# cmower/optas

Measured on AMD Instinct MI355X. Metric: MPC solves/sec (KUKA 7-DoF, T=50), higher is better.
Workload: dtype f64; 1 GPU; figure_eight_plan T=50 KUKA LWR end_effector_ball (BASELINE configs[1]) x 262144 perturbed instances per GPU (qc0 + U(-0.1,0.1)^7, seed=qc), solved to reduced-gradient tol 1e-08, max_iter 300; batch_per_gpu=262144, global_batch=262144, T=50, parallelism=dp1 (instances sharded, one RCCL broadcast of constants), rccl_world=1, hessian=hybrid, streams_per_gpu=2

## Files before the change

### optas_amd/csrc/oh_api.hip

```cpp
#include <dlfcn.h>
#include <hip/hip_runtime.h>
#include <rccl/rccl.h>

#include <chrono>
#include <cmath>
#include <cstdio>
#include <cstdlib>
#include <cstring>
#include <array>
#include <map>
#include <mutex>
#include <string>
#include <thread>
#include <utility>
#include <vector>

#include "oh_kernels.h"
#include "oh_jit.h"
#include "oh_rnea.h"

static thread_local std::string g_err;

static int fail(int code, const std::string& msg) {
  g_err = msg;
  return code;
}

#define HIPCHK(expr)                                                                                   \
  do {                                                                                                 \
    hipError_t _e = (expr);                                                                            \
    if (_e != hipSuccess) {                                                                            \
      return fail(OH_ERR_HIP, std::string(#expr) + ": " + hipGetErrorString(_e));                     \
    }                                                                                                  \
  } while (0)

#define OH_PINNED_STAGE_BYTES (256 * 1024)

struct Sched {
  int compaction = 1;
  int compact_carry = 1;
  int tail_vel_threshold = 1 << 30;
  int lg_split = 1;
  int tail_vel = 1;
  int compact_sort = 1;
  double compact_frac = 0.97;
  double compact_frac_restart = 0.9;
  int tail_threshold = 16384;
  int sparse_check_below = 2048;
  int fuse_couple = 1;
  int free_pcr_max = 1536;
  int specialize = OH_SPECIALIZE_AUTO;
  int tq_check = 4;
  std::array<double, 4> inv_saved{1.0, 16384.0, 1.0, -2.0};
};

struct oh_handle;
struct LastSolve {
  struct Part { const oh_handle* q; int n; };
  int B = 0;
  std::vector<Part> parts;
  bool pipe_cache = false;
};

// ... 57 lines not shown
  int cap_B = 0;
  FigBuffers D{};
  FigParams P{};
  void* pool = nullptr;
  size_t pool_bytes = 0;
  LastSolve last;
  void* stage = nullptr;
  size_t stage_bytes = 0;
  bool profiling = false;
  std::vector<hipEvent_t> prof_events;
  double timing[8] = {0, 0, 0, 0, 0, 0, 0, 0};
  double timing_couple = 0;
  double rejects = 0;
  double tail_iters = 0;
  int* h_flag = nullptr;
  std::vector<oh_handle*> peers;
  double* d_pipe_mult = nullptr;
  size_t pipe_mult_cap = 0;
  bool is_peer = false;
  Sched sch;
  int specialize_min_B = 4096;
  const FigSpec* spec = nullptr;
  bool spec_failed = false;
  bool spec_cache_checked = false;
  const FkSpec* fk_spec = nullptr;
  bool fk_spec_failed = false;
  int specialize_min_units = 1 << 16;
  double spec_seconds = 0.0;
  std::vector<int> prof_tags;
  std::map<std::string, double> opt;
  std::vector<int> t_op, t_a, t_b, t_rows;
  std::vector<double> t_c;
  oh_tape_desc t_desc{};
};

extern "C" void oh_destroy(oh_handle* h);
extern "C" int oh_specialize(oh_handle* h);
static bool spec_applies(const oh_handle* h);
static bool spec_tail_vel_applies(const oh_handle* h);
static int specialize_fk(oh_handle* h);
extern "C" const char* oh_last_error(void) { return g_err.c_str(); }
extern "C" const char* oh_version(void) { return "optas_hip 0.2 (gfx950)"; }
extern "C" int oh_abi_version(void) { return OH_ABI_VERSION; }

struct OptDoc { const char* name; double dflt; };
static constexpr OptDoc OPT_TABLE[] = {
// ... 17 lines not shown
  static_assert(ROW >= 0, "optv: the option is not in OPT_TABLE");
  return ROW;
}
static double opt_value(const oh_handle* h, const OptDoc& d) {
  const auto it = h->opt.find(d.name);
  return it == h->opt.end() ? d.dflt : it->second;
}
#define optv(h, name) opt_value(h, OPT_TABLE[known_opt<opt_row(name)>()])
static double batch_invariant(const oh_handle* h) {
  const auto it = h->opt.find("batch_invariant");
  return it == h->opt.end() ? 0.0 : it->second;
}
struct FieldOpt {
  const char* name;
  int Sched::*i;
  double Sched::*d = nullptr;
  bool flag = false;
  double get(const Sched& s) const { return d ? s.*d : s.*i; }
  void set(Sched& s, const double v) const { if (d) s.*d = v; else s.*i = flag ? v != 0.0 : (int)v; }
};
static const FieldOpt FIELD_OPTS[] = {
    {"tail_threshold", &Sched::tail_threshold}, {"free_pcr_max", &Sched::free_pcr_max}, {"compaction", &Sched::compaction, nullptr, true},
    {"compact_frac", nullptr, &Sched::compact_frac}, {"compact_sort", &Sched::compact_sort}, {"compact_carry", &Sched::compact_carry},
    {"tail_vel", &Sched::tail_vel}, {"lg_split", &Sched::lg_split}, {"tail_vel_threshold", &Sched::tail_vel_threshold},
    {"fuse_couple", &Sched::fuse_couple, nullptr, true}, {"sparse_check_below", &Sched::sparse_check_below}, {"specialize", &Sched::specialize},
    {"tq_check", &Sched::tq_check},
};
static const FieldOpt* field_opt(const std::string& name) {
  for (const FieldOpt& f : FIELD_OPTS)
    if (name == f.name) return &f;
  return nullptr;
}
static int tape_configure(oh_handle* h);
static int set_option_impl(oh_handle* h, const std::string& name, double v) {
  Sched& sc = h->sch;
  if (name == "compact_frac") sc.compact_frac = sc.compact_frac_restart = v;
  else if (name == "specialize") sc.specialize = v == 0.0 ? OH_SPECIALIZE_NEVER : (v == 1.0 ? OH_SPECIALIZE_ALWAYS : OH_SPECIALIZE_AUTO);
  else if (name == "tq_check") sc.tq_check = v >= 1.0 ? (int)v : 1;
  else if (name == "batch_invariant") {
    const bool was = batch_invariant(h) != 0.0;
    h->opt[name] = v;
    if (v != 0.0 && !was) {
      sc.inv_saved = {sc.compaction ? 1.0 : 0.0, (double)sc.tail_threshold, (double)sc.tail_vel, h->opt.count("free_persist") ? h->opt["free_persist"] : -2.0};
      sc.compaction = false; sc.tail_threshold = 0; sc.tail_vel = 0; h->opt["free_persist"] = 0;
    } else if (v == 0.0 && was) {
      sc.compaction = sc.inv_saved[0] != 0.0; sc.tail_threshold = (int)sc.inv_saved[1]; sc.tail_vel = (int)sc.inv_saved[2];
// ... 909 lines not shown
  if (c.n_chain < 1 || c.n_chain > OH_MAX_CHAIN || c.ndof < c.n_chain || c.ndof > OH_MAX_CHAIN)
    return fail(OH_ERR_INVALID, "oh_set_constants: bad n_chain/ndof");
  for (int k = 0; k < c.n_chain; ++k) {
    if (c.jtype[k] != 0 && c.jtype[k] != 1) return fail(OH_ERR_INVALID, "oh_set_constants: joint type not supported");
    if (c.qidx[k] < 0 || c.qidx[k] >= c.ndof) return fail(OH_ERR_INVALID, "oh_set_constants: qidx out of range");
  }
  if (c.ndof != h->desc.ndof) return fail(OH_ERR_INVALID, "oh_set_constants: chain.ndof != desc.ndof");
  return OH_OK;
}

static void drop_peers(oh_handle* h) {
  h->last = LastSolve{};
  if (h->is_peer) return;
  for (oh_handle* p : h->peers) oh_destroy(p);
  h->peers.clear();
}

static void adopt_chain(oh_handle* h, const oh_chain& c) {
  drop_peers(h);
  h->chain_host = c;
  h->have_chain = true;
  h->spec = nullptr;
  h->spec_failed = false;
  h->spec_cache_checked = false;
  h->fk_spec = nullptr;
  h->fk_spec_failed = false;
}

extern "C" int oh_set_constants(oh_handle* h, const oh_chain* chain) {
  if (!h || !chain) return fail(OH_ERR_INVALID, "oh_set_constants: null argument");
  int rc = validate_chain(h, *chain);
  if (rc) return rc;
  HIPCHK(hipMemcpy(h->d_chain, chain, sizeof(oh_chain), hipMemcpyHostToDevice));
  adopt_chain(h, *chain);
  return OH_OK;
}

extern "C" int oh_set_constants_device(oh_handle* h, const void* d_chain, size_t nbytes) {
  if (!h || !d_chain) return fail(OH_ERR_INVALID, "oh_set_constants_device: null argument");
  if (nbytes != sizeof(oh_chain)) return fail(OH_ERR_INVALID, "oh_set_constants_device: nbytes != sizeof(oh_chain)");
  oh_chain tmp;
  HIPCHK(hipMemcpy(&tmp, d_chain, sizeof(oh_chain), hipMemcpyDeviceToHost));
  int rc = validate_chain(h, tmp);
  if (rc) return rc;
  HIPCHK(hipMemcpy(h->d_chain, d_chain, sizeof(oh_chain), hipMemcpyDeviceToDevice));
  adopt_chain(h, tmp);
// ... 535 lines not shown
  const bool tail_vel = r.guarded && (GP.vel || GP.limits) && GP.n_links == 0 && h->sch.tail_vel;
  const bool tail_ok = (h->desc.T - P.t0 <= 64) && h->sch.tail_threshold > 0 && (!r.guarded || tail_vel) && !r.lead;
  const int tail_threshold = tail_vel ? h->sch.tail_vel_threshold : h->sch.tail_threshold;
  if (tail_ok && r.B <= tail_threshold) {
    if (!launch_tail(h, r, tail_vel, 0)) return fail(OH_ERR_INVALID, "oh_solve_device: no persistent kernel for this handle (ndof / rows)");
    return OH_OK;
  }
  const bool lg_split = r.guarded && h->sch.lg_split && GP.n_links == 0, lg_spec = lg_split && h->spec && spec_tail_vel_applies(h);
  const bool couple_vel = !P.zc && r.guarded && GP.vel, couple = !P.zc && !couple_vel;
  const bool carry = h->sch.compaction && h->sch.compact_carry && (size_t)h->desc.T * ((N - 3) * (N - 2) / 2) >= 22 && !r.guarded && !r.lead;
  const double inv_frac = optv(h, "invariant_compact_frac");
  const bool inv_move = r.invariant && !r.lead && inv_frac > 0.0, restart = h->sch.compaction && !r.lead, restart_moves = r.guarded && optv(h, "compact_move_all") != 0.0;
  int nrun = -1, carry_pending = 0;
  for (int it = 0; it < r.hard_cap; ++it) {
    if (nrun >= 0)
      if (const int rc = mark(h, r, 0, 3)) return rc;
    const int slot = it & 1;
    if (lg_split) {
      if (!(lg_spec && oh_spec_launch_eval(*h->spec, s, P, D, slot, 1) == hipSuccess)) oh_launch_eval_locked_guarded(s, N, P, D, GP, GB, slot, 1);
      oh_launch_eval_locked_guarded(s, N, P, D, GP, GB, slot, 2);
    } else if (r.guarded) oh_launch_eval_locked_guarded(s, N, P, D, GP, GB, slot, 0);
    else if (r.lead) oh_launch_eval_lead(s, N, P, D, slot);
    else if (carry_pending > 0) {
      launch_eval(h, r, slot, 1);
      if (const int rc = mark(h, r, 4)) return rc;
      finalize(h, r, 1);
      oh_launch_scan_running(s, D, h->sch.compact_sort);
      oh_launch_carry(s, N, P, D, 0, 0, slot);
      oh_launch_carry(s, N, P, D, 1, carry_pending, slot);
      std::swap(D.q[slot], D.q_spare[0]);
      std::swap(D.q[1 - slot], D.q_spare[1]);
      if (P.hessian != OH_HESSIAN_GAUSS_NEWTON || P.zc) std::swap(D.Gfull[1 - slot], D.G_spare);
      D.B = carry_pending;
      carry_pending = 0;
      ++r.compactions;
      if (const int rc = mark(h, r, 0)) return rc;
      launch_eval(h, r, slot, 2);
    } else launch_eval(h, r, slot, 0);
    if (const int rc = mark(h, r, 1)) return rc;
    if (couple_vel) oh_launch_couple_vel(s, N, P, D, GP, GB, slot);
    else if (couple) oh_launch_couple(s, N, P, D, slot);
    const bool check = check_after(h, r, it, tail_ok);
    if (const int rc = mark(h, r, 3)) return rc;
    if (r.guarded) oh_launch_step_locked_guarded(s, N, P, D, GP, GB, slot);
    else oh_launch_step(s, N, P, D, slot);
    if (const int rc = mark(h, r, 2)) return rc;
    ++r.launched;
    if (const int rc = look(h, check, &nrun)) return rc;
    if (nrun == 0) break;
    if (tail_ok && nrun > 0 && nrun <= tail_threshold) {
      if (const int rc = compact_batch(h, r, nrun, (it + 1) & 1, false)) return rc;
// ... 876 lines not shown
```

### optas_amd/csrc/oh_figure8_kernels.h

```cpp
#pragma once
#include "oh_figure8_units.h"

template <int N>
__device__ void retract_block(const FigParams& P, const FigBuffers& D, const int slot) {
  eval_unit<N, false, false, EVAL_RETRACT_ONLY>(P, D, slot, blockIdx.x * blockDim.x + threadIdx.x, blockIdx.y + P.t0);
}
template <int N>
__device__ void finalize_block(const FigParams& P, const FigBuffers& D, const int only_done, double* __restrict__ f, double* __restrict__ kkt, int* __restrict__ iters,
                               int* __restrict__ status) {
  finalize_unit<N>(P, D, only_done, nullptr, f, kkt, iters, status, blockIdx.x * blockDim.x + threadIdx.x, blockIdx.y);
}
template <int N, bool ZC = false>
__device__ void evalb_block(const FigParams& P, const FigBuffers& D, const int slot) {
  if constexpr (ZC) {
    if (blockIdx.x == 0 && threadIdx.x == 0) *D.n_running = 0;
    const int Tn = P.T - P.t0;
    const int w = blockIdx.x;
    const int chunk = w / (8 * Tn), r = w - chunk * 8 * Tn;
    eval_unit<N, false, false, EVAL_ONLY, true>(P, D, slot, (chunk * 8 + (r & 7)) * blockDim.x + threadIdx.x, (r >> 3) + P.t0);
  } else {
    eval_unit<N, false, false, EVAL_ONLY, false>(P, D, slot, blockIdx.x * blockDim.x + threadIdx.x, blockIdx.y + P.t0);
  }
}

OH_DEV double bcast(const double v, const int lane) {
  int lo = __double2loint(v), hi = __double2hiint(v);
  lo = __builtin_amdgcn_readlane(lo, lane);
  hi = __builtin_amdgcn_readlane(hi, lane);
// ... 523 lines not shown
```

### optas_amd/csrc/oh_figure8_units.h

```cpp
#pragma once
#include "oh_figure8.h"

#define IDX(t, K, k) (((size_t)(t) * (K) + (k)) * Bp + b)
#define KNOT(arr, t, K) rowbuf((arr) + (size_t)(t) * (K) * (size_t)Bp)
#define RB(k) ((unsigned)(k) * rowB)



template <int N>
OH_DEV void setup_unit(const FigParams& P, const FigBuffers& D, const double* __restrict__ x0, const double* __restrict__ pin, const int b, const int tt) {
  const int Bp = D.Bp;
  if (b >= D.B) {
    if (b < Bp && tt == 0) D.status[b] = OH_STATUS_CONVERGED;
    return;
  }
  const oh_chain* ch = D.chain;
  double qc[N];
#pragma unroll
  for (int j = 0; j < N; ++j) qc[j] = pin[(size_t)b * P.np + j];
#pragma unroll
  for (int j = 0; j < N; ++j) {
    const double v = (tt < P.t0) ? qc[j] : x0[(size_t)b * P.nx + (size_t)tt * N + j];
    D.q[0][IDX(tt, N, j)] = v;
    D.q[1][IDX(tt, N, j)] = (tt < P.t0) ? qc[j] : 0.0;
  }
  if (ch->has_lead) D.lead[(size_t)tt * Bp + b] = pin[(size_t)b * P.np + N + 1 + tt];
  if (tt != 0) return;
  double R[9], p[3], z[N][3], pj[N][3];
// ... 34 lines not shown
  D.feas[b] = 0.0;
}

#ifndef OH_CHAIN
#define OH_CHAIN(D) ((D).chain)
#endif
#ifndef OH_RETRACT_PREFETCH
#define OH_RETRACT_PREFETCH 0
#endif
#ifndef OH_EVALB_PREFETCH_G
#define OH_EVALB_PREFETCH_G 1
#endif
#ifndef OH_ZC_EARLY
#define OH_ZC_EARLY 1
#endif
template <int N>
OH_DEV void load_householder(const double* __restrict__ Vs, const int Bp, const int b, const int t, double (&V)[3][N]) {
#pragma unroll
  for (int m = 0; m < 3; ++m)
#pragma unroll
    for (int k = 0; k < N; ++k) V[m][k] = (k < m) ? 0.0 : Vs[IDX(t, HV_ROWS(N), HV_OFF(N, m) + k - m)];
}

template <int N, bool GUARD = false, bool LEAD = false, int MODE = EVAL_FUSED, bool ZC = false, bool SPH = true>
OH_DEV void eval_unit(const FigParams& P, const FigBuffers& D, const int slot, const int b, const int t, const GuardParams* GPp = nullptr,
                      const GuardBuffers* GBp = nullptr) {
  static_assert(!ZC || (MODE == EVAL_ONLY && !GUARD && !LEAD), "the folded coupling belongs to the plain batched evaluation");
  constexpr int NZ = N - 3;
  constexpr int NP = NZ * (NZ + 1) / 2;
  const int Bp = D.Bp;
  if (b >= D.B) return;
  const int cur = 1 - slot;
  const int status_b = D.status[b], skip_b = D.skip[b], first_b = D.first[b];
  const bool asis = (MODE == EVAL_RETRACT_ONLY && !GUARD) ? D.polish[b] == 2 : false;
  const double stat_b = D.stat[b], pred_b = D.pred[b];
  constexpr bool EARLY = MODE == EVAL_ONLY || OH_RETRACT_PREFETCH;
  double Rc[9], pc[3];
  if constexpr (EARLY) {
#pragma unroll
    for (int i = 0; i < 3; ++i) pc[i] = D.ref[(size_t)i * Bp + b];
#pragma unroll
    for (int i = 0; i < 9; ++i) Rc[i] = D.ref[(size_t)(3 + i) * Bp + b];
  }
  double q[N], e_tgt[3] = {0.0, 0.0, 0.0};
  double sm_zc = 0.0;
  double zs[NZ], Vc[3][N], mdlc[3 + 3 * NZ];
  double Gpre[N];
  constexpr bool PRE_G = OH_EVALB_PREFETCH_G && MODE == EVAL_ONLY && !GUARD;
  if constexpr (MODE == EVAL_ONLY) {
#pragma unroll
    for (int j = 0; j < N; ++j) q[j] = D.q[slot][IDX(t, N, j)];
    if constexpr (PRE_G) {
      if (P.hessian != OH_HESSIAN_GAUSS_NEWTON) {
#pragma unroll
        for (int k = 0; k < N; ++k) Gpre[k] = D.Gfull[cur][IDX(t, N, k)];
      }
    }
  } else if constexpr (OH_RETRACT_PREFETCH) {
#pragma unroll
    for (int a = 0; a < NZ; ++a) zs[a] = D.zstep[IDX(t, NZ, a)];
    load_householder<N>(D.Z[cur], Bp, b, t, Vc);
#pragma unroll
    for (int j = 0; j < N; ++j) q[j] = D.q[cur][IDX(t, N, j)];
#pragma unroll
    for (int i = 0; i < 3 + 3 * NZ; ++i) mdlc[i] = D.mdl[cur][IDX(t, MDL_ROWS(N), i)];
  }
  double cpl_zc[N];
  if constexpr (ZC && OH_ZC_EARLY) {
    const double* __restrict__ qs = D.q[slot];
    const bool lastk = (t == P.T - 1);
    double qm[N], qp[N];
#pragma unroll
    for (int k = 0; k < N; ++k) {
      qm[k] = qs[IDX(t - 1, N, k)];
      qp[k] = lastk ? 0.0 : qs[IDX(t + 1, N, k)];
    }
    oh_fence(q[N - 1]);
    oh_fence(Rc[8]);
    oh_fence(qp[N - 1]);
    const double kap2 = 2.0 * P.kappa;
#pragma unroll
    for (int k = 0; k < N; ++k) {
      const double dm = q[k] - qm[k];
      sm_zc += dm * dm;
      double c = kap2 * dm;
      if (!lastk) c -= kap2 * (qp[k] - q[k]);
      cpl_zc[k] = c;
    }
  } else if constexpr (EARLY) {
    oh_fence(q[N - 1]);
    oh_fence(Rc[8]);
  }
  if (status_b >= 0 || skip_b) return;
  const bool first = first_b != 0;
  if constexpr (MODE != EVAL_ONLY) {
    if (first) {
#pragma unroll
      for (int j = 0; j < N; ++j) q[j] = D.q[slot][IDX(t, N, j)];
    } else {
      if constexpr (!OH_RETRACT_PREFETCH) {
#pragma unroll
        for (int a = 0; a < NZ; ++a) zs[a] = D.zstep[IDX(t, NZ, a)];
        load_householder<N>(D.Z[cur], Bp, b, t, Vc);
#pragma unroll
        for (int j = 0; j < N; ++j) q[j] = D.q[cur][IDX(t, N, j)];
#pragma unroll
        for (int i = 0; i < 3 + 3 * NZ; ++i) mdlc[i] = D.mdl[cur][IDX(t, MDL_ROWS(N), i)];
      }
      double Zc[N][NZ];
      z_from_householder<N>(Vc, Zc);
#pragma unroll
      for (int j = 0; j < N; ++j) {
        double v = q[j];
#pragma unroll
        for (int a = 0; a < NZ; ++a) v += Zc[j][a] * zs[a];
        q[j] = asis ? q[j] : v;
      }
#pragma unroll
      for (int m = 0; m < 3; ++m) {
        double v = mdlc[m];
#pragma unroll
        for (int a = 0; a < NZ; ++a) v += mdlc[3 + m * NZ + a] * zs[a];
        e_tgt[m] = v;
      }
    }
  }
  if constexpr (!EARLY) {
#pragma unroll
    for (int i = 0; i < 3; ++i) pc[i] = D.ref[(size_t)i * Bp + b];
#pragma unroll
    for (int i = 0; i < 9; ++i) Rc[i] = D.ref[(size_t)(3 + i) * Bp + b];
  }
  double Gprev[N];
  const bool fresh = first_b == 1;
  bool exact = (P.hessian == OH_HESSIAN_EXACT) || (P.hessian == OH_HESSIAN_HYBRID && !fresh && stat_b <= P.hyb_switch);
  if constexpr (GUARD) {
    if (SPH && GPp->n_links > 0) exact = false;
  }
  const bool have_G = exact && !fresh;
#pragma unroll
  for (int k = 0; k < N; ++k) Gprev[k] = 0.0;

  double phi, cv, g[N], Dr[NP], Z[N][NZ];
  struct Hooks {
    double* __restrict__ qo;
    double* __restrict__ go;
    double* __restrict__ vo;
    const double* __restrict__ Gc;
    int Bp, b, t;
    OH_DEV void q_final(const double (&qv)[N]) const {
      if constexpr (!GUARD && MODE != EVAL_ONLY) {
#pragma unroll
        for (int j = 0; j < N; ++j) qo[IDX(t, N, j)] = qv[j];
      }
    }
    OH_DEV void g_final(const double (&gv)[N]) const {
      if constexpr (ZC && OH_ZC_EARLY) {
#pragma unroll
        for (int k = 0; k < N; ++k) Go[IDX(t, N, k)] = gv[k] + cpl[k];
      } else if constexpr (ZC) {
        double sm = 0.0;
#pragma unroll
        for (int k = 0; k < N; ++k) {
          const double q0 = qr[k];
          const double dm = q0 - qs[IDX(t - 1, N, k)];
          sm += dm * dm;
          double Gk = gv[k] + kap2 * dm;
          if (!last) Gk -= kap2 * (qs[IDX(t + 1, N, k)] - q0);
          Go[IDX(t, N, k)] = Gk;
        }
        *smo = sm;
      } else if constexpr (!GUARD) {
#pragma unroll
        for (int k = 0; k < N; ++k) go[IDX(t, N, k)] = gv[k];
      }
    }
    OH_DEV void v_final(const double (&Vv)[3][N]) const {
#pragma unroll
      for (int m = 0; m < 3; ++m)
#pragma unroll
        for (int k = m; k < N; ++k) vo[IDX(t, HV_ROWS(N), HV_OFF(N, m) + k - m)] = Vv[m][k];
    }
    const double* Gp;
    OH_DEV void load_G(const double (&)[N], double (&G)[N]) const {
#pragma unroll
      for (int k = 0; k < N; ++k) G[k] = PRE_G ? Gp[k] : Gc[IDX(t, N, k)];
    }
    const double* __restrict__ qs;
    const double* qr;
    double* __restrict__ Go;
    double* smo;
    double kap2;
    bool last;
    const double* cpl;
  };
  const Hooks hooks{D.q[slot], D.g[slot], D.Z[slot], D.Gfull[cur], Bp, b, t, Gpre, D.q[slot], q, D.Gfull[slot], &sm_zc, 2.0 * P.kappa, t == P.T - 1, cpl_zc};
  double e_new[3], JZ_new[3][NZ];
  const double tol_r = (first_b == 2 || asis) ? 1e300 : retract_tol(P, !first, pred_b, stat_b);
  if constexpr (LEAD)
    eval_knot<N, true, Hooks, MODE>(OH_CHAIN(D), P, t, q, pc, Rc, exact, have_G, Gprev, phi, cv, g, Dr, Z, !first, e_tgt, tol_r, e_new, JZ_new,
                                    D.lead[(size_t)t * Bp + b], hooks);
  else eval_knot<N, false, Hooks, MODE>(OH_CHAIN(D), P, t, q, pc, Rc, exact, have_G, Gprev, phi, cv, g, Dr, Z, !first, e_tgt, tol_r, e_new, JZ_new, 0.0, hooks);
  if constexpr (MODE == EVAL_RETRACT_ONLY) return;
#pragma unroll
  for (int m = 0; m < 3; ++m) {
    D.mdl[slot][IDX(t, MDL_ROWS(N), m)] = e_new[m];
#pragma unroll
    for (int a = 0; a < NZ; ++a) D.mdl[slot][IDX(t, MDL_ROWS(N), 3 + m * NZ + a)] = JZ_new[m][a];
  }
  if constexpr (GUARD) {
    const GuardParams& GP = *GPp;
    const GuardBuffers& GB = *GBp;
    const bool upd = GB.outer[b] != 0;
    const double rho_old = GB.rho[b];
    const double rho = upd ? GB.rho_next[b] : rho_old;
    const double irho = 1.0 / rho, i2rho = 1.0 / (2.0 * rho);
    double psi = 0.0, meas = 0.0, dd[N];
    const int nl = GP.limits ? 2 * N : 0;
#pragma unroll
// ... 866 lines not shown
```

### optas_amd/csrc/oh_jit.h

```cpp
#pragma once
#include <string>
#include <vector>

#include "oh_kernels.h"

struct FigSpec {
  hipModule_t mod = nullptr;
  hipFunction_t retract = nullptr, evalb = nullptr, evalb_zc = nullptr, tail = nullptr, tail_vel = nullptr, finalize = nullptr;
  int n = 0;
  bool from_disk = false;
  double seconds = 0.0;
};
std::string oh_jit_figure8_source(const oh_chain& chain, int N);
int oh_jit_compile_cached(const std::string& src, std::vector<char>* code, bool* from_disk, std::string* err, bool ignore_disk = false);
int oh_jit_figure8(const oh_chain& chain, int N, const FigSpec** out, std::string* err);
bool oh_jit_figure8_cached(const oh_chain& chain, int N);
hipError_t oh_spec_launch_eval(const FigSpec& sp, hipStream_t s, const FigParams& P, const FigBuffers& D, int slot, int part);
hipError_t oh_spec_launch_tail(const FigSpec& sp, hipStream_t s, const FigParams& P, const FigBuffers& D, int slot);
hipError_t oh_spec_launch_finalize(const FigSpec& sp, hipStream_t s, FigParams P, FigBuffers D, int only_done, double* f, double* kkt, int* iters, int* status);
hipError_t oh_spec_launch_tail_vel(const FigSpec& sp, hipStream_t s, FigParams P, FigBuffers D, GuardParams GP, GuardBuffers GB, int slot);
bool oh_spec_kernel_info(const FigSpec& sp, const char* name, OhKernelInfo* out);

bool oh_jit_disk_lookup(const std::string& key_text, const char* prefix, std::vector<char>* code);
void oh_jit_disk_store(const std::string& key_text, const char* prefix, const std::vector<char>& code);
void oh_jit_disk_drop(const std::string& key_text, const char* prefix);

struct FkSpec {
  hipModule_t mod = nullptr;
  hipFunction_t soa = nullptr, aos = nullptr;
  int ndof = 0;
  bool from_disk = false;
// ... 7 lines not shown
```

### optas_amd/csrc/oh_jit.hip

```cpp
#include <hip/hip_runtime.h>
#include <hip/hiprtc.h>
#include <sys/stat.h>
#include <unistd.h>

#include <chrono>
#include <cstdio>
#include <cstdlib>
#include <cstring>
#include <map>
#include <mutex>
#include <string>
#include <vector>

#include "oh_jit.h"
#include "oh_fkjac_unit.h"
#include "oh_jit_headers.h"

namespace {
std::mutex g_mutex;
std::map<unsigned long long, FigSpec*> g_specs;
std::map<unsigned long long, FkSpec*> g_fk_specs;

unsigned long long fnv1a(const std::string& s, unsigned long long h = 1469598103934665603ull) {
  for (unsigned char c : s) {
// ... 151 lines not shown
  char name[96];
  snprintf(name, sizeof name, "%s_%016llx.hsaco", prefix, fnv1a("hiprtc " + std::to_string(major) + "." + std::to_string(minor), fnv1a(key_text)));
  remove((dir + "/" + name).c_str());
}

std::string oh_jit_figure8_source(const oh_chain& chain, int N) {
  std::string s;
  s += "// generated by liboptas_hip (oh_jit.hip): figure-eight evaluation kernels for one kinematic chain\n";
  s += "#include \"oh_types.h\"\n";
  s += "static __device__ constexpr oh_chain oh_spec_chain = " + chain_literal(chain) + ";\n";
  s += "#define OH_CHAIN(D) (&oh_spec_chain)\n";
#ifndef OH_JIT_RETRACT_PREFETCH
#define OH_JIT_RETRACT_PREFETCH 1
#endif
  s += "#define OH_RETRACT_PREFETCH " + std::to_string(OH_JIT_RETRACT_PREFETCH) + "\n";
#ifndef OH_JIT_ZC_EARLY
#define OH_JIT_ZC_EARLY 1
#endif
  s += "#define OH_ZC_EARLY " + std::to_string(OH_JIT_ZC_EARLY) + "\n";
  s += "#include \"oh_platform_gfx950.h\"\n";
  s += "#include \"oh_figure8_kernels.h\"\n";
  const std::string n = std::to_string(N);
  s += "extern \"C\" __global__ __launch_bounds__(256, 2) void oh_spec_retract(FigParams P, FigBuffers D, const int slot) { retract_block<" + n + ">(P, D, slot); }\n";
  s += "extern \"C\" __global__ __launch_bounds__(256, 2) void oh_spec_evalb(FigParams P, FigBuffers D, const int slot) { evalb_block<" + n + ">(P, D, slot); }\n";
  s += "extern \"C\" __global__ __launch_bounds__(256, 2) void oh_spec_evalb_zc(FigParams P, FigBuffers D, const int slot) { evalb_block<" + n + ", true>(P, D, slot); }\n";
  s += "extern \"C\" __global__ __launch_bounds__(64) void oh_spec_tail(FigParams P, FigBuffers D, const int slot) { tail_block<" + n + ">(P, D, slot); }\n";
  s += "extern \"C\" __global__ __launch_bounds__(256) void oh_spec_finalize(FigParams P, FigBuffers D, const int only_done, double* f, double* kkt, int* iters, int* status) { finalize_block<" + n +
       ">(P, D, only_done, f, kkt, iters, status); }\n";
  s += "extern \"C\" __global__ __launch_bounds__(64) void oh_spec_tail_vel(FigParams P, FigBuffers D, GuardParams GP, GuardBuffers GB, const int slot) { tail_block<" + n +
       ", true>(P, D, slot, &GP, &GB); }\n";
  return s;
}

int oh_jit_compile_cached(const std::string& src, std::vector<char>* code, bool* from_disk, std::string* err, bool ignore_disk) {
  const std::string name = cache_name(src);
  const std::string dir = cache_dir();
  *from_disk = false;
  if (ignore_disk && !dir.empty()) remove((dir + "/" + name).c_str());
  if (!ignore_disk && !dir.empty() && read_file(dir + "/" + name, code)) {
    *from_disk = true;
    return 0;
  }
  if (compile(src, code, err)) return 1;
  if (!dir.empty()) {
    mkdirs(dir);
    write_file_atomic(dir + "/" + name, *code);
// ... 22 lines not shown
  const auto t0 = std::chrono::steady_clock::now();
  const std::string src = oh_jit_figure8_source(chain, N);
  int dev = 0;
  hipGetDevice(&dev);
  const unsigned long long key = fnv1a(src) ^ (0x9e3779b97f4a7c15ull * (unsigned long long)(dev + 1));
  std::lock_guard<std::mutex> lk(g_mutex);
  auto it = g_specs.find(key);
  if (it != g_specs.end()) {
    *out = it->second;
    return 0;
  }
  std::vector<char> code;
  bool from_disk = false;
  FigSpec* sp = new FigSpec();
  for (int attempt = 0;; ++attempt) {
    if (oh_jit_compile_cached(src, &code, &from_disk, err, attempt > 0)) {
      delete sp;
      return 1;
    }
    const char* what = nullptr;
    if (hipModuleLoadData(&sp->mod, code.data()) != hipSuccess) what = "hipModuleLoadData";
    else if (hipModuleGetFunction(&sp->retract, sp->mod, "oh_spec_retract") != hipSuccess || hipModuleGetFunction(&sp->evalb, sp->mod, "oh_spec_evalb") != hipSuccess ||
             hipModuleGetFunction(&sp->tail, sp->mod, "oh_spec_tail") != hipSuccess || hipModuleGetFunction(&sp->evalb_zc, sp->mod, "oh_spec_evalb_zc") != hipSuccess ||
             hipModuleGetFunction(&sp->tail_vel, sp->mod, "oh_spec_tail_vel") != hipSuccess || hipModuleGetFunction(&sp->finalize, sp->mod, "oh_spec_finalize") != hipSuccess) {
      what = "hipModuleGetFunction";
      hipModuleUnload(sp->mod);
    }
    if (!what) break;
    (void)hipGetLastError();
    if (from_disk && attempt == 0) continue;
    *err = std::string(what) + " failed for the specialised figure-eight kernels";
    delete sp;
    return 1;
  }
  sp->n = N;
  sp->from_disk = from_disk;
  sp->seconds = std::chrono::duration<double>(std::chrono::steady_clock::now() - t0).count();
  g_specs.emplace(key, sp);
  *out = sp;
  return 0;
}

static hipError_t launch3(hipFunction_t f, dim3 g, dim3 b, hipStream_t s, FigParams P, FigBuffers D, int slot) {
  void* args[] = {&P, &D, &slot};
  return hipModuleLaunchKernel(f, g.x, g.y, g.z, b.x, b.y, b.z, 0, s, args, nullptr);
}
hipError_t oh_spec_launch_eval(const FigSpec& sp, hipStream_t s, const FigParams& P, const FigBuffers& D, int slot, int part) {
  const dim3 ge((D.B + 255) / 256, P.T - P.t0);
  hipError_t e = hipSuccess;
  if (part != 2) e = launch3(sp.retract, ge, dim3(256), s, P, D, slot);
  if (e == hipSuccess && part != 1) {
    if (P.zc) e = launch3(sp.evalb_zc, dim3((((D.B + 255) / 256) + 7) / 8 * 8 * (P.T - P.t0)), dim3(256), s, P, D, slot);
    else e = launch3(sp.evalb, ge, dim3(256), s, P, D, slot);
  }
  return e;
}
hipError_t oh_spec_launch_tail(const FigSpec& sp, hipStream_t s, const FigParams& P, const FigBuffers& D, int slot) {
  return launch3(sp.tail, dim3(D.B), dim3(64), s, P, D, slot);
}
hipError_t oh_spec_launch_finalize(const FigSpec& sp, hipStream_t s, FigParams P, FigBuffers D, int only_done, double* f, double* kkt, int* iters, int* status) {
  void* args[] = {&P, &D, &only_done, &f, &kkt, &iters, &status};
  return hipModuleLaunchKernel(sp.finalize, (D.B + 255) / 256, D.lam_h ? P.T : 1, 1, 256, 1, 1, 0, s, args, nullptr);
}
hipError_t oh_spec_launch_tail_vel(const FigSpec& sp, hipStream_t s, FigParams P, FigBuffers D, GuardParams GP, GuardBuffers GB, int slot) {
  void* args[] = {&P, &D, &GP, &GB, &slot};
  return hipModuleLaunchKernel(sp.tail_vel, D.B, 1, 1, 64, 1, 1, 0, s, args, nullptr);
}
bool oh_spec_kernel_info(const FigSpec& sp, const char* name, OhKernelInfo* out) {
  const std::string n(name);
  hipFunction_t f = n == "k_retract" ? sp.retract : n == "k_evalb" ? sp.evalb : n == "k_evalb_zc" ? sp.evalb_zc : n == "k_tail" ? sp.tail : n == "k_tail_vel" ? sp.tail_vel : nullptr;
  if (!f) return false;
  int v = 0, sc = 0, lds = 0;
  if (hipFuncGetAttribute(&v, HIP_FUNC_ATTRIBUTE_NUM_REGS, f) != hipSuccess) return false;
  hipFuncGetAttribute(&sc, HIP_FUNC_ATTRIBUTE_LOCAL_SIZE_BYTES, f);
  hipFuncGetAttribute(&lds, HIP_FUNC_ATTRIBUTE_SHARED_SIZE_BYTES, f);
  out->vgprs = v;
  out->scratch_bytes = sc;
  out->lds_bytes = lds;
  out->block = (n == "k_tail" || n == "k_tail_vel") ? 64 : 256;
  int nb = 0;
  if (hipModuleOccupancyMaxActiveBlocksPerMultiprocessor(&nb, f, out->block, 0) != hipSuccess) nb = 0;
  out->blocks_per_cu = nb;
  return true;
}

std::string oh_jit_fkjac_source(const oh_chain& chain) {
  std::string s;
  s += "// generated by liboptas_hip (oh_jit.hip): forward kinematics + geometric Jacobian for one kinematic chain\n";
  s += "#include \"oh_fkjac_unit.h\"\n";
  s += "static __device__ constexpr oh_chain oh_spec_chain = " + chain_literal(chain) + ";\n";
  const std::string nc = std::to_string(chain.n_chain);
  for (int soa = 0; soa < 2; ++soa)
    s += std::string("extern \"C\" __global__ __launch_bounds__(256) void oh_spec_fk_") + (soa ? "soa" : "aos") +
// ... 61 lines not shown
```

### optas_amd/csrc/oh_kernels.hip

```cpp
#include "oh_platform_gfx950.h"
#include "oh_figure8_kernels.h"
#include "oh_kernels.h"

#define OH_DISPATCH_N(n, call)         \
  switch (n) {                         \
    case 4: call(4); break;            \
    case 5: call(5); break;            \
    case 6: call(6); break;            \
    case 7: call(7); break;            \
    case 8: call(8); break;            \
    default: return false;             \
  }
#define OH_DISPATCH_N_ANY(n, call)     \
  switch (n) {                         \
    case 2: call(2); break;            \
    case 3: call(3); break;            \
    case 4: call(4); break;            \
    case 5: call(5); break;            \
    case 6: call(6); break;            \
    case 7: call(7); break;            \
    case 8: call(8); break;            \
    default: return false;             \
  }

// ... 282 lines not shown
    D.q[slot][IDX(t, N, j)] = v;
    if (t < P.t0) D.q[1 - slot][IDX(t, N, j)] = v;
    if (P.hessian != OH_HESSIAN_GAUSS_NEWTON || P.zc) D.Gfull[1 - slot][IDX(t, N, j)] = D.g[1][IDX(t, N, j)];
  }
  if (t == 0) {
#pragma unroll
    for (int i = 0; i < 12; ++i) D.ref[(size_t)i * Bp + b] = ts[(size_t)i * Bp + b];
    D.fconst[b] = ts[(size_t)12 * Bp + b];
    D.mu[b] = ts[(size_t)13 * Bp + b];
    D.nun[b] = ts[(size_t)16 * Bp + b];
    const int it = (int)ts[(size_t)14 * Bp + b];
    D.iters[b] = it > 0 ? it - 1 : 0;
    D.orig[b] = (int)ts[(size_t)15 * Bp + b];
    D.cur[b] = 1 - slot;
    D.stat[b] = ts[(size_t)17 * Bp + b];
    D.first[b] = 2;
    D.skip[b] = 0;
    D.polish[b] = 0;
    D.stale[b] = 0;
    D.status[b] = -1;
  }
}

template <int N>
__global__ __launch_bounds__(256) void k_carry_gather(FigParams P, FigBuffers D, const int slot) {
  const int b = blockIdx.x * blockDim.x + threadIdx.x;
  const int t = blockIdx.y;
  const int Bp = D.Bp;
  if (b >= D.B) return;
  const int nb = D.newidx[b];
  if (nb < 0) return;
  const bool restart = D.skip[b] != 0 || D.first[b] != 0;
  const int cur = restart ? slot : 1 - slot;
  double* __restrict__ t_trial = D.q_spare[0];
  double* __restrict__ t_cur = D.q_spare[1];
  double* __restrict__ t_G = D.G_spare;
  double* __restrict__ ts = D.Dr[1];
#pragma unroll
  for (int j = 0; j < N; ++j) {
    t_trial[((size_t)t * N + j) * Bp + nb] = D.q[slot][IDX(t, N, j)];
    t_cur[((size_t)t * N + j) * Bp + nb] = D.q[cur][IDX(t, N, j)];
    if (P.hessian != OH_HESSIAN_GAUSS_NEWTON || P.zc) t_G[((size_t)t * N + j) * Bp + nb] = D.Gfull[cur][IDX(t, N, j)];
  }
  if (t == 0) {
#pragma unroll
    for (int i = 0; i < 12; ++i) ts[(size_t)i * Bp + nb] = D.ref[(size_t)i * Bp + b];
    ts[(size_t)12 * Bp + nb] = D.fconst[b];
    ts[(size_t)13 * Bp + nb] = D.mu[b];
    ts[(size_t)14 * Bp + nb] = (double)(D.iters[b] - ((D.skip[b] != 0 && D.first[b] == 0) ? 1 : 0));
    ts[(size_t)15 * Bp + nb] = (double)D.orig[b];
    ts[(size_t)16 * Bp + nb] = D.nun[b];
    ts[(size_t)17 * Bp + nb] = D.f_cur[b];
    ts[(size_t)18 * Bp + nb] = D.pred[b];
    ts[(size_t)19 * Bp + nb] = D.stat[b];
    ts[(size_t)20 * Bp + nb] = D.feas[b];
    ts[(size_t)21 * Bp + nb] = (double)((restart ? 1 : 0) + 2 * (D.polish[b] != 0 ? 1 : 0) + 4 * (D.polish[b] == 2 ? 1 : 0));
  }
}
template <int N>
__global__ __launch_bounds__(256) void k_carry_scatter(FigParams P, FigBuffers D, int Bnew, const int slot) {
  const int b = blockIdx.x * blockDim.x + threadIdx.x;
  const int Bp = D.Bp;
  if (b >= Bnew) return;
  const double* __restrict__ ts = D.Dr[1];
  {
// ... 16 lines not shown
    D.skip[b] = 0;
    D.polish[b] = (!restart && (flags & 2)) ? ((flags & 4) ? 2 : 1) : 0;
    D.stale[b] = restart ? 0 : 1;
    D.status[b] = -1;
  }
}

template <int N>
static void launch_setup_t(hipStream_t s, const FigParams& P, const FigBuffers& D, const double* x0, const double* p) {
  hipLaunchKernelGGL(k_setup<N>, dim3((D.B + 63) / 64, P.T), dim3(64), 0, s, P, D, x0, p);
}
template <int N>
static void launch_eval_t(hipStream_t s, const FigParams& P, const FigBuffers& D, int slot, int part) {
  const dim3 ge((D.B + 255) / 256, P.T - P.t0);
  if (part != 2) hipLaunchKernelGGL(k_retract<N>, ge, dim3(256), 0, s, P, D, slot);
  if (part != 1) {
    if (P.zc) hipLaunchKernelGGL(k_evalb_zc<N>, dim3((((D.B + 255) / 256) + 7) / 8 * 8 * (P.T - P.t0)), dim3(256), 0, s, P, D, slot);
    else hipLaunchKernelGGL(k_evalb<N>, ge, dim3(256), 0, s, P, D, slot);
  }
}
template <int N>
static void launch_carry_t(hipStream_t s, const FigParams& P, const FigBuffers& D, int phase, int Bnew, int slot) {
  if (phase == 0) hipLaunchKernelGGL(k_carry_gather<N>, dim3((D.B + 255) / 256, P.T), dim3(256), 0, s, P, D, slot);
  else hipLaunchKernelGGL(k_carry_scatter<N>, dim3((Bnew + 255) / 256), dim3(256), 0, s, P, D, Bnew, slot);
}
template <int N>
static void launch_couple_t(hipStream_t s, const FigParams& P, const FigBuffers& D, int slot) {
  const int nbx8 = (((D.B + 255) / 256) + 7) / 8 * 8;
  hipLaunchKernelGGL(k_couple<N>, dim3(nbx8 * (P.T - P.t0)), dim3(256), 0, s, P, D, slot);
}
template <int N>
static void launch_step_t(hipStream_t s, const FigParams& P, const FigBuffers& D, int slot) {
  if (P.zc) {
    hipLaunchKernelGGL(k_step_zc<N>, dim3((D.B + 63) / 64), dim3(64), 0, s, P, D, slot);
    if (P.hessian != OH_HESSIAN_GAUSS_NEWTON) hipLaunchKernelGGL(k_defer_copy<N>, dim3(512), dim3(256), 0, s, P, D, slot);
  } else hipLaunchKernelGGL(k_step<N>, dim3((D.B + 63) / 64), dim3(64), 0, s, P, D, slot);
}
template <int N>
static void launch_tail_t(hipStream_t s, const FigParams& P, const FigBuffers& D, int slot) {
  hipLaunchKernelGGL(k_tail<N>, dim3(D.B), dim3(64), 0, s, P, D, slot);
}
template <int N>
__global__ __launch_bounds__(256) void k_finalize_x(FigParams P, FigBuffers D, const int only_done, double* __restrict__ x) {
  constexpr int TK = 8, ROWS = (TK + 1) * N;
  __shared__ double tile[ROWS][65];
  __shared__ long long orig_s[64];
// ... 184 lines not shown
```

Measured before the change: 2.983 million solves/s.

## Fuse compaction gather into specialized retraction kernel on carry iterations

On iterations with a pending compaction carry, the finalize and running scan now run before the retraction. A new JIT-specialized retraction variant then writes q trial/current and G directly into the compacted spare buffers at their new indices. The full carry-gather pass over all timesteps shrinks to a small gather covering only rows before t0 plus the per-instance scalar state, which removes a full read/write of the q and G arrays. This reorders finalize and scan ahead of the retraction and adds another specialized kernel. If the kernel is unavailable, the old path is used.

```diff
diff --git a/optas_amd/csrc/oh_api.hip b/optas_amd/csrc/oh_api.hip
--- a/optas_amd/csrc/oh_api.hip
+++ b/optas_amd/csrc/oh_api.hip
@@ -39,6 +39,7 @@
 struct Sched {
   int compaction = 1;
   int compact_carry = 1;
+  int compact_fused = 1;
   int tail_vel_threshold = 1 << 30;
   int lg_split = 1;
   int tail_vel = 1;
@@ -142,6 +143,7 @@
   int specialize_min_B = 4096;
   const FigSpec* spec = nullptr;
   bool spec_failed = false;
+  bool spec_move_failed = false;
   bool spec_cache_checked = false;
   const FkSpec* fk_spec = nullptr;
   bool fk_spec_failed = false;
@@ -205,6 +207,7 @@
 static const FieldOpt FIELD_OPTS[] = {
     {"tail_threshold", &Sched::tail_threshold}, {"free_pcr_max", &Sched::free_pcr_max}, {"compaction", &Sched::compaction, nullptr, true},
     {"compact_frac", nullptr, &Sched::compact_frac}, {"compact_sort", &Sched::compact_sort}, {"compact_carry", &Sched::compact_carry},
+    {"compact_fused", &Sched::compact_fused, nullptr, true},
     {"tail_vel", &Sched::tail_vel}, {"lg_split", &Sched::lg_split}, {"tail_vel_threshold", &Sched::tail_vel_threshold},
     {"fuse_couple", &Sched::fuse_couple, nullptr, true}, {"sparse_check_below", &Sched::sparse_check_below}, {"specialize", &Sched::specialize},
     {"tq_check", &Sched::tq_check},
@@ -1160,6 +1163,7 @@
   h->have_chain = true;
   h->spec = nullptr;
   h->spec_failed = false;
+  h->spec_move_failed = false;
   h->spec_cache_checked = false;
   h->fk_spec = nullptr;
   h->fk_spec_failed = false;
@@ -1741,11 +1745,30 @@
     } else if (r.guarded) oh_launch_eval_locked_guarded(s, N, P, D, GP, GB, slot, 0);
     else if (r.lead) oh_launch_eval_lead(s, N, P, D, slot);
     else if (carry_pending > 0) {
-      launch_eval(h, r, slot, 1);
-      if (const int rc = mark(h, r, 4)) return rc;
-      finalize(h, r, 1);
-      oh_launch_scan_running(s, D, h->sch.compact_sort);
-      oh_launch_carry(s, N, P, D, 0, 0, slot);
+      bool moved = false, scanned = false;
+      if (r.spec && r.spec->retract_move && h->sch.compact_fused && !h->spec_move_failed) {
+        finalize(h, r, 1);
+        oh_launch_scan_running(s, D, h->sch.compact_sort);
+        scanned = true;
+        if (const int rc = mark(h, r, 0)) return rc;
+        moved = oh_spec_launch_eval(*r.spec, s, P, D, slot, 3) == hipSuccess;
+        if (moved) {
+          if (const int rc = mark(h, r, 4)) return rc;
+          oh_launch_carry(s, N, P, D, 2, 0, slot);
+        } else {
+          (void)hipGetLastError();
+          h->spec_move_failed = true;
+        }
+      }
+      if (!moved) {
+        launch_eval(h, r, slot, 1);
+        if (const int rc = mark(h, r, 4)) return rc;
+        if (!scanned) {
+          finalize(h, r, 1);
+          oh_launch_scan_running(s, D, h->sch.compact_sort);
+        }
+        oh_launch_carry(s, N, P, D, 0, 0, slot);
+      }
       oh_launch_carry(s, N, P, D, 1, carry_pending, slot);
       std::swap(D.q[slot], D.q_spare[0]);
       std::swap(D.q[1 - slot], D.q_spare[1]);
diff --git a/optas_amd/csrc/oh_figure8_kernels.h b/optas_amd/csrc/oh_figure8_kernels.h
--- a/optas_amd/csrc/oh_figure8_kernels.h
+++ b/optas_amd/csrc/oh_figure8_kernels.h
@@ -1,9 +1,9 @@
 #pragma once
 #include "oh_figure8_units.h"
 
-template <int N>
+template <int N, bool MOVE = false>
 __device__ void retract_block(const FigParams& P, const FigBuffers& D, const int slot) {
-  eval_unit<N, false, false, EVAL_RETRACT_ONLY>(P, D, slot, blockIdx.x * blockDim.x + threadIdx.x, blockIdx.y + P.t0);
+  eval_unit<N, false, false, EVAL_RETRACT_ONLY, false, true, MOVE>(P, D, slot, blockIdx.x * blockDim.x + threadIdx.x, blockIdx.y + P.t0);
 }
 template <int N>
 __device__ void finalize_block(const FigParams& P, const FigBuffers& D, const int only_done, double* __restrict__ f, double* __restrict__ kkt, int* __restrict__ iters,
diff --git a/optas_amd/csrc/oh_figure8_units.h b/optas_amd/csrc/oh_figure8_units.h
--- a/optas_amd/csrc/oh_figure8_units.h
+++ b/optas_amd/csrc/oh_figure8_units.h
@@ -4,6 +4,7 @@
 #define IDX(t, K, k) (((size_t)(t) * (K) + (k)) * Bp + b)
 #define KNOT(arr, t, K) rowbuf((arr) + (size_t)(t) * (K) * (size_t)Bp)
 #define RB(k) ((unsigned)(k) * rowB)
+#define SPARE(k) (((size_t)t * N + (k)) * Bp + nb)
 
 
 
@@ -84,10 +85,11 @@
     for (int k = 0; k < N; ++k) V[m][k] = (k < m) ? 0.0 : Vs[IDX(t, HV_ROWS(N), HV_OFF(N, m) + k - m)];
 }
 
-template <int N, bool GUARD = false, bool LEAD = false, int MODE = EVAL_FUSED, bool ZC = false, bool SPH = true>
+template <int N, bool GUARD = false, bool LEAD = false, int MODE = EVAL_FUSED, bool ZC = false, bool SPH = true, bool MOVE = false>
 OH_DEV void eval_unit(const FigParams& P, const FigBuffers& D, const int slot, const int b, const int t, const GuardParams* GPp = nullptr,
                       const GuardBuffers* GBp = nullptr) {
   static_assert(!ZC || (MODE == EVAL_ONLY && !GUARD && !LEAD), "the folded coupling belongs to the plain batched evaluation");
+  static_assert(!MOVE || (MODE == EVAL_RETRACT_ONLY && !GUARD && !LEAD), "the moving retraction belongs to the plain batched retraction");
   constexpr int NZ = N - 3;
   constexpr int NP = NZ * (NZ + 1) / 2;
   const int Bp = D.Bp;
@@ -96,6 +98,10 @@
   const int status_b = D.status[b], skip_b = D.skip[b], first_b = D.first[b];
   const bool asis = (MODE == EVAL_RETRACT_ONLY && !GUARD) ? D.polish[b] == 2 : false;
   const double stat_b = D.stat[b], pred_b = D.pred[b];
+  int nb = 0;
+  if constexpr (MOVE) nb = D.newidx[b];
+  const bool move_G = MOVE && (P.hessian != OH_HESSIAN_GAUSS_NEWTON || P.zc);
+  double Gmv[N];
   constexpr bool EARLY = MODE == EVAL_ONLY || OH_RETRACT_PREFETCH;
   double Rc[9], pc[3];
   if constexpr (EARLY) {
@@ -126,6 +132,12 @@
     for (int j = 0; j < N; ++j) q[j] = D.q[cur][IDX(t, N, j)];
 #pragma unroll
     for (int i = 0; i < 3 + 3 * NZ; ++i) mdlc[i] = D.mdl[cur][IDX(t, MDL_ROWS(N), i)];
+    if constexpr (MOVE) {
+      if (move_G) {
+#pragma unroll
+        for (int k = 0; k < N; ++k) Gmv[k] = D.Gfull[cur][IDX(t, N, k)];
+      }
+    }
   }
   double cpl_zc[N];
   if constexpr (ZC && OH_ZC_EARLY) {
@@ -153,12 +165,35 @@
     oh_fence(q[N - 1]);
     oh_fence(Rc[8]);
   }
-  if (status_b >= 0 || skip_b) return;
+  if constexpr (MOVE) {
+    if (status_b >= 0 || nb < 0) return;
+    if (skip_b) {
+#pragma unroll
+      for (int j = 0; j < N; ++j) {
+        const double v = D.q[slot][IDX(t, N, j)];
+        D.q_spare[0][SPARE(j)] = v;
+        D.q_spare[1][SPARE(j)] = v;
+      }
+      if (move_G) {
+#pragma unroll
+        for (int k = 0; k < N; ++k) D.G_spare[SPARE(k)] = D.Gfull[slot][IDX(t, N, k)];
+      }
+      return;
+    }
+  } else {
+    if (status_b >= 0 || skip_b) return;
+  }
   const bool first = first_b != 0;
   if constexpr (MODE != EVAL_ONLY) {
     if (first) {
 #pragma unroll
       for (int j = 0; j < N; ++j) q[j] = D.q[slot][IDX(t, N, j)];
+      if constexpr (MOVE) {
+        if (move_G) {
+#pragma unroll
+          for (int k = 0; k < N; ++k) D.G_spare[SPARE(k)] = D.Gfull[slot][IDX(t, N, k)];
+        }
+      }
     } else {
       if constexpr (!OH_RETRACT_PREFETCH) {
 #pragma unroll
@@ -168,6 +203,20 @@
         for (int j = 0; j < N; ++j) q[j] = D.q[cur][IDX(t, N, j)];
 #pragma unroll
         for (int i = 0; i < 3 + 3 * NZ; ++i) mdlc[i] = D.mdl[cur][IDX(t, MDL_ROWS(N), i)];
+        if constexpr (MOVE) {
+          if (move_G) {
+#pragma unroll
+            for (int k = 0; k < N; ++k) Gmv[k] = D.Gfull[cur][IDX(t, N, k)];
+          }
+        }
+      }
+      if constexpr (MOVE) {
+#pragma unroll
+        for (int j = 0; j < N; ++j) D.q_spare[1][SPARE(j)] = q[j];
+        if (move_G) {
+#pragma unroll
+          for (int k = 0; k < N; ++k) D.G_spare[SPARE(k)] = Gmv[k];
+        }
       }
       double Zc[N][NZ];
       z_from_householder<N>(Vc, Zc);
@@ -211,7 +260,14 @@
     const double* __restrict__ Gc;
     int Bp, b, t;
     OH_DEV void q_final(const double (&qv)[N]) const {
-      if constexpr (!GUARD && MODE != EVAL_ONLY) {
+      if constexpr (MOVE) {
+#pragma unroll
+        for (int j = 0; j < N; ++j) qo[SPARE(j)] = qv[j];
+        if (qo2) {
+#pragma unroll
+          for (int j = 0; j < N; ++j) qo2[SPARE(j)] = qv[j];
+        }
+      } else if constexpr (!GUARD && MODE != EVAL_ONLY) {
 #pragma unroll
         for (int j = 0; j < N; ++j) qo[IDX(t, N, j)] = qv[j];
       }
@@ -255,8 +311,11 @@
     double kap2;
     bool last;
     const double* cpl;
+    double* __restrict__ qo2;
+    int nb;
   };
-  const Hooks hooks{D.q[slot], D.g[slot], D.Z[slot], D.Gfull[cur], Bp, b, t, Gpre, D.q[slot], q, D.Gfull[slot], &sm_zc, 2.0 * P.kappa, t == P.T - 1, cpl_zc};
+  const Hooks hooks{MOVE ? D.q_spare[0] : D.q[slot], D.g[slot], D.Z[slot], D.Gfull[cur], Bp, b, t, Gpre, D.q[slot], q, D.Gfull[slot], &sm_zc, 2.0 * P.kappa, t == P.T - 1, cpl_zc,
+                    (MOVE && first) ? D.q_spare[1] : nullptr, nb};
   double e_new[3], JZ_new[3][NZ];
   const double tol_r = (first_b == 2 || asis) ? 1e300 : retract_tol(P, !first, pred_b, stat_b);
   if constexpr (LEAD)
diff --git a/optas_amd/csrc/oh_jit.h b/optas_amd/csrc/oh_jit.h
--- a/optas_amd/csrc/oh_jit.h
+++ b/optas_amd/csrc/oh_jit.h
@@ -6,7 +6,7 @@
 
 struct FigSpec {
   hipModule_t mod = nullptr;
-  hipFunction_t retract = nullptr, evalb = nullptr, evalb_zc = nullptr, tail = nullptr, tail_vel = nullptr, finalize = nullptr;
+  hipFunction_t retract = nullptr, retract_move = nullptr, evalb = nullptr, evalb_zc = nullptr, tail = nullptr, tail_vel = nullptr, finalize = nullptr;
   int n = 0;
   bool from_disk = false;
   double seconds = 0.0;
diff --git a/optas_amd/csrc/oh_jit.hip b/optas_amd/csrc/oh_jit.hip
--- a/optas_amd/csrc/oh_jit.hip
+++ b/optas_amd/csrc/oh_jit.hip
@@ -197,6 +197,7 @@
   s += "#include \"oh_figure8_kernels.h\"\n";
   const std::string n = std::to_string(N);
   s += "extern \"C\" __global__ __launch_bounds__(256, 2) void oh_spec_retract(FigParams P, FigBuffers D, const int slot) { retract_block<" + n + ">(P, D, slot); }\n";
+  s += "extern \"C\" __global__ __launch_bounds__(256, 2) void oh_spec_retract_move(FigParams P, FigBuffers D, const int slot) { retract_block<" + n + ", true>(P, D, slot); }\n";
   s += "extern \"C\" __global__ __launch_bounds__(256, 2) void oh_spec_evalb(FigParams P, FigBuffers D, const int slot) { evalb_block<" + n + ">(P, D, slot); }\n";
   s += "extern \"C\" __global__ __launch_bounds__(256, 2) void oh_spec_evalb_zc(FigParams P, FigBuffers D, const int slot) { evalb_block<" + n + ", true>(P, D, slot); }\n";
   s += "extern \"C\" __global__ __launch_bounds__(64) void oh_spec_tail(FigParams P, FigBuffers D, const int slot) { tail_block<" + n + ">(P, D, slot); }\n";
@@ -265,7 +266,8 @@
     if (hipModuleLoadData(&sp->mod, code.data()) != hipSuccess) what = "hipModuleLoadData";
     else if (hipModuleGetFunction(&sp->retract, sp->mod, "oh_spec_retract") != hipSuccess || hipModuleGetFunction(&sp->evalb, sp->mod, "oh_spec_evalb") != hipSuccess ||
              hipModuleGetFunction(&sp->tail, sp->mod, "oh_spec_tail") != hipSuccess || hipModuleGetFunction(&sp->evalb_zc, sp->mod, "oh_spec_evalb_zc") != hipSuccess ||
-             hipModuleGetFunction(&sp->tail_vel, sp->mod, "oh_spec_tail_vel") != hipSuccess || hipModuleGetFunction(&sp->finalize, sp->mod, "oh_spec_finalize") != hipSuccess) {
+             hipModuleGetFunction(&sp->tail_vel, sp->mod, "oh_spec_tail_vel") != hipSuccess || hipModuleGetFunction(&sp->finalize, sp->mod, "oh_spec_finalize") != hipSuccess ||
+             hipModuleGetFunction(&sp->retract_move, sp->mod, "oh_spec_retract_move") != hipSuccess) {
       what = "hipModuleGetFunction";
       hipModuleUnload(sp->mod);
     }
@@ -291,6 +293,7 @@
 hipError_t oh_spec_launch_eval(const FigSpec& sp, hipStream_t s, const FigParams& P, const FigBuffers& D, int slot, int part) {
   const dim3 ge((D.B + 255) / 256, P.T - P.t0);
   hipError_t e = hipSuccess;
+  if (part == 3) return launch3(sp.retract_move, ge, dim3(256), s, P, D, slot);
   if (part != 2) e = launch3(sp.retract, ge, dim3(256), s, P, D, slot);
   if (e == hipSuccess && part != 1) {
     if (P.zc) e = launch3(sp.evalb_zc, dim3((((D.B + 255) / 256) + 7) / 8 * 8 * (P.T - P.t0)), dim3(256), s, P, D, slot);
@@ -311,7 +314,7 @@
 }
 bool oh_spec_kernel_info(const FigSpec& sp, const char* name, OhKernelInfo* out) {
   const std::string n(name);
-  hipFunction_t f = n == "k_retract" ? sp.retract : n == "k_evalb" ? sp.evalb : n == "k_evalb_zc" ? sp.evalb_zc : n == "k_tail" ? sp.tail : n == "k_tail_vel" ? sp.tail_vel : nullptr;
+  hipFunction_t f = n == "k_retract" ? sp.retract : n == "k_retract_move" ? sp.retract_move : n == "k_evalb" ? sp.evalb : n == "k_evalb_zc" ? sp.evalb_zc : n == "k_tail" ? sp.tail : n == "k_tail_vel" ? sp.tail_vel : nullptr;
   if (!f) return false;
   int v = 0, sc = 0, lds = 0;
   if (hipFuncGetAttribute(&v, HIP_FUNC_ATTRIBUTE_NUM_REGS, f) != hipSuccess) return false;
diff --git a/optas_amd/csrc/oh_kernels.hip b/optas_amd/csrc/oh_kernels.hip
--- a/optas_amd/csrc/oh_kernels.hip
+++ b/optas_amd/csrc/oh_kernels.hip
@@ -328,7 +328,7 @@
   }
 }
 
-template <int N>
+template <int N, bool REST = false>
 __global__ __launch_bounds__(256) void k_carry_gather(FigParams P, FigBuffers D, const int slot) {
   const int b = blockIdx.x * blockDim.x + threadIdx.x;
   const int t = blockIdx.y;
@@ -342,11 +342,13 @@
   double* __restrict__ t_cur = D.q_spare[1];
   double* __restrict__ t_G = D.G_spare;
   double* __restrict__ ts = D.Dr[1];
-#pragma unroll
-  for (int j = 0; j < N; ++j) {
-    t_trial[((size_t)t * N + j) * Bp + nb] = D.q[slot][IDX(t, N, j)];
-    t_cur[((size_t)t * N + j) * Bp + nb] = D.q[cur][IDX(t, N, j)];
-    if (P.hessian != OH_HESSIAN_GAUSS_NEWTON || P.zc) t_G[((size_t)t * N + j) * Bp + nb] = D.Gfull[cur][IDX(t, N, j)];
+  if (!REST || t < P.t0) {
+#pragma unroll
+    for (int j = 0; j < N; ++j) {
+      t_trial[((size_t)t * N + j) * Bp + nb] = D.q[slot][IDX(t, N, j)];
+      t_cur[((size_t)t * N + j) * Bp + nb] = D.q[cur][IDX(t, N, j)];
+      if (P.hessian != OH_HESSIAN_GAUSS_NEWTON || P.zc) t_G[((size_t)t * N + j) * Bp + nb] = D.Gfull[cur][IDX(t, N, j)];
+    }
   }
   if (t == 0) {
 #pragma unroll
@@ -409,6 +411,7 @@
 template <int N>
 static void launch_carry_t(hipStream_t s, const FigParams& P, const FigBuffers& D, int phase, int Bnew, int slot) {
   if (phase == 0) hipLaunchKernelGGL(k_carry_gather<N>, dim3((D.B + 255) / 256, P.T), dim3(256), 0, s, P, D, slot);
+  else if (phase == 2) hipLaunchKernelGGL((k_carry_gather<N, true>), dim3((D.B + 255) / 256, P.t0 > 1 ? P.t0 : 1), dim3(256), 0, s, P, D, slot);
   else hipLaunchKernelGGL(k_carry_scatter<N>, dim3((Bnew + 255) / 256), dim3(256), 0, s, P, D, Bnew, slot);
 }
 template <int N>
```

Result: faster. 3.077 million solves/s (median of 6 runs) (+3.2%).
